# jkk-research/urban_road_filter

Measured on NVIDIA H100. Metric: scans_per_sec, higher is better.
Workload: dtype f32/f64

## Files before the change

### urban_road_filter_b200/csrc/urf_api.cu

```cuda
#include <algorithm>
#include <cmath>
#include <cstdio>
#include <cstdlib>
#include <cstring>
#include <string>
#include <vector>

#include "urf_kernels.cuh"
#include "urf_host.hpp"

using namespace urf;

struct urf_ctx {
  int device = 0;
  int max_points = 0;
  int max_batch = 0;
  size_t P = 0;
  int Tmax = 0;
  cudaStream_t stream = nullptr;
  cudaStream_t s_in = nullptr, s_out = nullptr;
  static constexpr int kGroups = 16;
  cudaStream_t s_grp[kGroups] = {};
  cudaEvent_t ev_fork = nullptr, ev_join[kGroups] = {};
  cudaStream_t s_side[kGroups + 1] = {};
  cudaEvent_t ev_sfork[kGroups + 1] = {}, ev_sjoin[kGroups + 1] = {};
  int sort_ctas = 0;
  int groups = 2;
  bool use_graph = true;
  cudaGraphExec_t gexec = nullptr;
  int g_B = -1, g_S = -1, g_order = -1, g_launches = 0;
  unsigned long long g_version = 0, version = 1;
  std::vector<cudaEvent_t> ev_in, ev_comp;
  cudaEvent_t ev0 = nullptr, ev1 = nullptr;
  DevBuffers buf{};
  float4* own_in = nullptr;
  unsigned char* rawb = nullptr;
  size_t rawb_bytes = 0;
  signed char* label8 = nullptr;
  int* own_label = nullptr;
  float4* pack = nullptr;
  int* packcnt = nullptr;
  int* packtot = nullptr;
  int* h_packtot = nullptr;
  urf_params params{};
  DevParams dp{};
  int* h_n = nullptr;
  static constexpr int kNRing = 8;
  int* h_nring = nullptr;
  cudaEvent_t ev_nring[kNRing] = {};
  int nring_pos = 0;
  ScanOut* h_out = nullptr;
  int last_B = 0, last_S = 0;
  int launches = 0;
  float last_ms = 0.f;
  bool timing_valid = false;
  std::string err;
  std::vector<void*> allocs;
  bool profile = false;
  int kslots = 1, kslot = 0;
  std::vector<cudaEvent_t> kev;
  std::vector<const char*> knames;
  std::vector<int> kcounts;
  int kcount = 0;
};

namespace {

int cuda_rc(urf_ctx* ctx, cudaError_t e, const char* call) {
  if (e == cudaSuccess) return URF_OK;
  ctx->err = std::string(call) + ": " + cudaGetErrorString(e);
  return e == cudaErrorMemoryAllocation ? URF_ERR_NOMEM : URF_ERR_CUDA;
}

#define CK(call)                                                                                   \
  do {                                                                                             \
    const int rc_ = cuda_rc(ctx, (call), #call);                                                   \
    if (rc_ != URF_OK) return rc_;                                                                 \
  } while (0)

template <class T> int dalloc(urf_ctx* ctx, T** p, size_t count) {
  void* q = nullptr;
  CK(cudaMalloc(&q, count * sizeof(T) + 256));
  ctx->allocs.push_back(q);
  CK(cudaMemsetAsync(q, 0, count * sizeof(T) + 256, ctx->stream));
  CK(cudaStreamSynchronize(ctx->stream));
  *p = static_cast<T*>(q);
  return URF_OK;
}

__global__ void k_ring32(DevBuffers buf, int* dst, int S) {
  const int b = blockIdx.y, i = blockIdx.x * blockDim.x + threadIdx.x;
  if (i < buf.n[b]) dst[(size_t)b * S + i] = max((int)buf.ringid[(size_t)b * S + i], -1);
}

DevBuffers offset_view(const DevBuffers& a, int b0, int S, int T, int channels) {
  DevBuffers v = a;
  const size_t o = (size_t)b0 * S;
  v.in += o; v.label += o; v.order += o; v.n += b0; v.out += b0;
  if (v.label8) v.label8 += o;
  v.alpha_v += o; v.mark += o; v.ringid += o; v.sect += o; v.bpt += o;
  v.sr += o; v.sz += o; v.sidx += o; v.ssrz += o; v.ssl += o;
  v.az += o; v.d2 += o; v.baz += o; v.roadlist += o; v.roadcnt += (size_t)b0 * ((S + 31) >> 5); v.sortbuf += 2 * o;
  v.Tf += (size_t)b0 * channels * kTStride; v.Tb += (size_t)b0 * channels * kTStride;
  v.lut += (size_t)b0 * (kElevBins + 1); v.firstidx += (size_t)b0 * (kElevBins + 1);
  v.hist += (size_t)b0 * T * kRingKeys;
  v.cmin += (size_t)b0 * channels * kDegBins; v.cmax += (size_t)b0 * channels * kDegBins;
  v.ne += (size_t)b0 * channels * (kDegBins + 1);
  v.tab += b0;
  return v;
}

constexpr int kMaxKernels = 32;
constexpr int kMarkSingleMax = 300000;
thread_local std::string g_create_err;

int launch_pipeline(urf_ctx* ctx, const DevBuffers& buf, int B, int S, bool want_order, int group, int* launched) {
  DevParams dp = ctx->dp;
  dp.want_order = want_order ? 1 : 0;
  cudaStream_t st = group < urf_ctx::kGroups ? ctx->s_grp[group] : ctx->stream;
  const int T = (S + kChunk - 1) / kChunk;
  if (T > ctx->Tmax) return URF_ERR_CAPACITY;
  int L = 0;
  ctx->kcount = 0;
  const dim3 gpts((S + 255) / 256, B), gchunk((T + kWarpsPerBlock - 1) / kWarpsPerBlock, B);
#define K(name, ...)                                                                         \
  do {                                                                                       \
    if (ctx->profile && ctx->kcount < kMaxKernels) {                                         \
      ctx->knames[ctx->kcount] = name;                                                       \
      CK(cudaEventRecord(ctx->kev[(size_t)ctx->kslot * (kMaxKernels + 1) + ctx->kcount], st)); \
      ctx->kcount++;                                                                         \
    }                                                                                        \
    __VA_ARGS__;                                                                             \
    L++;                                                                                     \
  } while (0)
  K("k_reset", k_reset<<<dim3(8, B), 256, 0, st>>>(buf, dp));
  K("k_points", k_points<<<gpts, 256, 0, st>>>(buf, dp, S));
  K("k_register", k_register<<<B, 256, 0, st>>>(buf, dp, S));
  K("k_assign", k_assign<<<gchunk, kWarpsPerBlock * 32, 0, st>>>(buf, dp, S, T));
  K("k_scan_offsets", k_scan_offsets<<<B, 1024, 0, st>>>(buf, dp, S, T));
  K("k_scatter", k_scatter<<<dim3((T + kScatterWarps - 1) / kScatterWarps, B), kScatterWarps * 32, kScatterSmem, st>>>(buf, dp, S, T));
  const bool fork = dp.star && !ctx->profile;
  cudaStream_t st_ring = fork ? ctx->s_side[group] : st;
  if (fork) {
    CK(cudaEventRecord(ctx->ev_sfork[group], st));
    CK(cudaStreamWaitEvent(st_ring, ctx->ev_sfork[group], 0));
  }
  if (dp.curbPoints == 5)
    K("k_ring_detect4", k_ring_detect4<<<dim3((S + kTile4 - 1) / kTile4, B), 256, 0, st_ring>>>(buf, dp, S));
  else K("k_ring_detect", k_ring_detect<<<gpts, 256, 0, st_ring>>>(buf, dp, S));
  if (fork) CK(cudaEventRecord(ctx->ev_sjoin[group], st_ring));
  if (dp.star) {
    const int gbig = std::max(4, std::min(kSectKeys, 2048 / B));
    const dim3 gscan((kSectKeys + kScanWarps * 32 - 1) / (kScanWarps * 32), B);
    const int gsort = std::min(ctx->sort_ctas, (B * kSectKeys + kSortWarps - 1) / kSortWarps);
    K("k_star_sort", k_star_sort<<<gsort, kSortWarps * 32, kStarSortSmem, st>>>(buf, dp, S, B));
    K("k_star_sort_big", k_star_sort_big<<<dim3(gbig, B), 256, kStarCtaSmem, st>>>(buf, dp, S));
    K("k_star_scan", k_star_scan<<<gscan, kScanWarps * 32, 0, st>>>(buf, dp, S));
    if (dp.star_prefix)
      K("k_star_refine", k_star_refine<<<dim3(std::max(8, std::min(kSectKeys / 8, 8192 / B)), B), 256, kStarCtaSmem, st>>>(buf, dp, S));
  }
  if (fork) CK(cudaStreamWaitEvent(st, ctx->ev_sjoin[group], 0));
  K("k_tab1", k_tab1<<<dim3((dp.channels + 7) / 8, B), 256, 0, st>>>(buf, dp));
  K("k_reach", k_reach<<<dim3((2 * kDegBins + 7) / 8, B), 256, 0, st>>>(buf, dp));
  K("k_tab2", k_tab2<<<dim3((dp.channels + kTab2Rings - 1) / kTab2Rings, B), kTab2Rings * 64, 0, st>>>(buf, dp));
  K("k_label", k_label<<<dim3((S + kLabelThreads * kLabelGroups - 1) / (kLabelThreads * kLabelGroups), B), kLabelThreads, 0, st>>>(buf, dp, S));
  if (S > kMarkSingleMax) {
    const dim3 gm(std::max(1, std::min(64, S / 16384)), B);
    K("k_markers_grid1", k_markers_grid<1><<<gm, kMarkGridThreads, 0, st>>>(buf, S));
    K("k_markers_grid2", k_markers_grid<2><<<gm, kMarkGridThreads, 0, st>>>(buf, S));
    K("k_verts", k_verts<<<B, 384, 0, st>>>(buf, S));
  } else K("k_markers1", k_markers1<<<dim3(1, B), kMark1Threads, 0, st>>>(buf, S));
  if (want_order) K("k_sort_rings", k_sort_rings<<<dim3(dp.channels, B), kSortThreads, kRingSmemKeys * sizeof(unsigned long long), st>>>(buf, S));
#undef K
  if (ctx->profile) {
    CK(cudaEventRecord(ctx->kev[(size_t)ctx->kslot * (kMaxKernels + 1) + kMaxKernels], st));
    ctx->kcounts[ctx->kslot] = ctx->kcount;
    ctx->kslot = (ctx->kslot + 1) % ctx->kslots;
  }
  CK(cudaGetLastError());
  *launched = L;
  return URF_OK;
}

int update_graph(urf_ctx* ctx, int B, int S, bool want_order) {
  if (ctx->gexec && ctx->g_B == B && ctx->g_S == S && ctx->g_order == (int)want_order && ctx->g_version == ctx->version) return URF_OK;
  if (ctx->gexec) { cudaGraphExecDestroy(ctx->gexec); ctx->gexec = nullptr; }
  cudaGraph_t graph = nullptr;
  CK(cudaStreamBeginCapture(ctx->stream, cudaStreamCaptureModeThreadLocal));
  int L = 0;
  const int rc = launch_pipeline(ctx, ctx->buf, B, S, want_order, urf_ctx::kGroups, &L);
  const cudaError_t e = cudaStreamEndCapture(ctx->stream, &graph);
  if (rc != URF_OK || e != cudaSuccess || !graph) { if (graph) cudaGraphDestroy(graph); ctx->err = "graph capture failed"; return rc != URF_OK ? rc : URF_ERR_CUDA; }
  const cudaError_t ei = cudaGraphInstantiate(&ctx->gexec, graph, 0);
  cudaGraphDestroy(graph);
  if (ei != cudaSuccess) { ctx->gexec = nullptr; ctx->err = cudaGetErrorString(ei); return URF_ERR_CUDA; }
  ctx->g_B = B; ctx->g_S = S; ctx->g_order = (int)want_order; ctx->g_version = ctx->version; ctx->g_launches = L;
  return URF_OK;
}

void fill_result(const ScanOut& o, urf_result* r, bool with_ring_start) {
  r->n_in = o.n_in; r->n_roi = o.n_roi;
  r->flags = o.flags & F_PUBLIC_MASK; r->reserved = 0;
  if (o.n_roi < 30) {
    r->status = URF_TOO_FEW_POINTS;
    r->n_rings = 0; r->n_order = 0; r->n_road = 0; r->n_curb = 0; r->n_vert = 0;
    if (with_ring_start && r->ring_start) for (int k = 0; k <= URF_MAX_CHANNELS; k++) r->ring_start[k] = 0;
    return;
  }
  r->status = URF_OK;
  r->n_rings = o.n_rings; r->n_order = o.n_order; r->n_road = o.n_road; r->n_curb = o.n_curb; r->n_vert = o.n_vert;
  std::memcpy(r->vert, o.vert, sizeof(float) * 4 * (size_t)o.n_vert);
  if (with_ring_start && r->ring_start) std::memcpy(r->ring_start, o.ring_start, sizeof(int) * (URF_MAX_CHANNELS + 1));
}

}

extern "C" {

int urf_version(void) { return URF_VERSION; }

const char* urf_strerror(int code) {
  switch (code) {
    case URF_OK: return "ok";
    case URF_TOO_FEW_POINTS: return "fewer than 30 points in the ROI: nothing published";
    case URF_ERR_INVALID: return "invalid argument";
    case URF_ERR_NO_DEVICE: return "no CUDA device (this library has no CPU fallback)";
    case URF_ERR_CUDA: return "CUDA error";
    case URF_ERR_NOMEM: return "out of device or pinned memory";
    case URF_ERR_CAPACITY: return "scan or batch larger than the context was created for";
    case URF_ERR_TIMEOUT: return "timed out";
    case URF_ERR_CLOSED: return "queue closed";
    default: return "unknown error";
  }
}

const char* urf_last_cuda_error(const urf_ctx* ctx) {
  if (ctx) return ctx->err.c_str();
  return g_create_err.empty() ? "null context" : g_create_err.c_str();
}

void urf_default_params(urf_params* p) {
  if (!p) return;
  std::memset(p, 0, sizeof(*p));
  std::snprintf(p->fixed_frame, sizeof(p->fixed_frame), "left_os1/os1_lidar");
  std::snprintf(p->topic_name, sizeof(p->topic_name), "/left_os1/os1_cloud_node/points");
  p->x_zero_method = 1; p->z_zero_method = 1; p->star_shaped_method = 1; p->blind_spots = 1; p->xDirection = 0;
  p->interval = 0.18; p->curb_height = 0.05; p->curb_points = 5; p->beamZone = 30;
  p->min_x = 0; p->max_x = 30; p->min_y = -10; p->max_y = 10; p->min_z = -3; p->max_z = -1;
  p->cylinder_deg_x = 150; p->cylinder_deg_z = 140; p->curb_slope_deg = 50;
  p->kdev_param = 1.225; p->kdist_param = 2; p->starbeam_filter = 0; p->dmin_param = 10;
  p->simple_poly_allow = 1; p->poly_s_param = 0.7; p->poly_z_manual = -1.5; p->poly_z_avg_allow = 1;
  p->channels = 64;
}

int urf_create(urf_ctx** out, int device, int max_points, int max_batch) {
  if (!out || max_points < 1 || max_batch < 1 || max_points > (1 << 24)) return URF_ERR_INVALID;
  if ((long long)(max_points + kChunk) * max_batch >= (1ll << 31)) return URF_ERR_CAPACITY;
  *out = nullptr;
  int ndev = 0;
  if (cudaGetDeviceCount(&ndev) != cudaSuccess || ndev <= 0 || device < 0 || device >= ndev) return URF_ERR_NO_DEVICE;
  urf_ctx* ctx = new urf_ctx();
  auto fail = [&](int rc) { g_create_err = ctx->err.empty() ? std::string(urf_strerror(rc)) : ctx->err; urf_destroy(ctx); return rc; };
  ctx->device = device;
  if (cudaSetDevice(device) != cudaSuccess) return fail(URF_ERR_NO_DEVICE);
  ctx->max_points = ((max_points + kChunk - 1) / kChunk) * kChunk;
  ctx->max_batch = max_batch;
  ctx->P = (size_t)ctx->max_points * max_batch;
  ctx->Tmax = ctx->max_points / kChunk;
  int rc;
#define TRY(x) do { rc = (x); if (rc != URF_OK) return fail(rc); } while (0)
#define CKF(call) do { cudaError_t e_ = (call); if (e_ != cudaSuccess) { ctx->err = cudaGetErrorString(e_); return fail(URF_ERR_CUDA); } } while (0)
  CKF(cudaStreamCreateWithFlags(&ctx->stream, cudaStreamNonBlocking));
  CKF(cudaStreamCreateWithFlags(&ctx->s_in, cudaStreamNonBlocking));
  CKF(cudaStreamCreateWithFlags(&ctx->s_out, cudaStreamNonBlocking));
  for (int g = 0; g < urf_ctx::kGroups; g++) {
    CKF(cudaStreamCreateWithFlags(&ctx->s_grp[g], cudaStreamNonBlocking));
    CKF(cudaEventCreateWithFlags(&ctx->ev_join[g], cudaEventDisableTiming));
  }
  CKF(cudaEventCreateWithFlags(&ctx->ev_fork, cudaEventDisableTiming));
  for (int g = 0; g <= urf_ctx::kGroups; g++) {
    CKF(cudaStreamCreateWithFlags(&ctx->s_side[g], cudaStreamNonBlocking));
    CKF(cudaEventCreateWithFlags(&ctx->ev_sfork[g], cudaEventDisableTiming));
    CKF(cudaEventCreateWithFlags(&ctx->ev_sjoin[g], cudaEventDisableTiming));
  }
  CKF(cudaEventCreate(&ctx->ev0));
  CKF(cudaEventCreate(&ctx->ev1));
  const size_t P = ctx->P;
  DevBuffers& b = ctx->buf;
  TRY(dalloc(ctx, &ctx->own_in, P));
  ctx->rawb_bytes = (size_t)ctx->max_points * URF_MAX_POINT_STEP;
  TRY(dalloc(ctx, &ctx->rawb, ctx->rawb_bytes));
  TRY(dalloc(ctx, &b.alpha_v, P));
  TRY(dalloc(ctx, &b.mark, P));
  TRY(dalloc(ctx, &b.ringid, P));
  TRY(dalloc(ctx, &b.sect, P));
  TRY(dalloc(ctx, &ctx->own_label, P));
  TRY(dalloc(ctx, &b.bpt, P));
  TRY(dalloc(ctx, &b.sr, P));
  TRY(dalloc(ctx, &b.sz, P));
  TRY(dalloc(ctx, &b.sidx, P));
  TRY(dalloc(ctx, &b.ssrz, P));
  TRY(dalloc(ctx, &b.ssl, P));
  TRY(dalloc(ctx, &b.az, P));
  TRY(dalloc(ctx, &b.d2, P));
  TRY(dalloc(ctx, &b.baz, P));
  TRY(dalloc(ctx, &b.roadlist, P));
  TRY(dalloc(ctx, &b.roadcnt, P / 32 + (size_t)max_batch + 1));
  TRY(dalloc(ctx, &b.Tf, (size_t)max_batch * kTStride * URF_MAX_CHANNELS));
  TRY(dalloc(ctx, &b.Tb, (size_t)max_batch * kTStride * URF_MAX_CHANNELS));
  TRY(dalloc(ctx, &b.lut, (size_t)max_batch * (kElevBins + 1)));
  TRY(dalloc(ctx, &b.order, P));
  TRY(dalloc(ctx, &b.sortbuf, 2 * P));
  TRY(dalloc(ctx, &b.hist, (size_t)max_batch * ctx->Tmax * kRingKeys));
  TRY(dalloc(ctx, &b.firstidx, (size_t)max_batch * (kElevBins + 1)));
  TRY(dalloc(ctx, &b.cmin, (size_t)max_batch * URF_MAX_CHANNELS * kDegBins));
  TRY(dalloc(ctx, &b.cmax, (size_t)max_batch * URF_MAX_CHANNELS * kDegBins));
  TRY(dalloc(ctx, &b.ne, (size_t)max_batch * URF_MAX_CHANNELS * (kDegBins + 1)));
  TRY(dalloc(ctx, &b.newY, (size_t)ctx->max_points));
  TRY(dalloc(ctx, &b.n, (size_t)max_batch));
  TRY(dalloc(ctx, &b.out, (size_t)max_batch));
  TRY(dalloc(ctx, &b.tab, (size_t)max_batch));
  b.in = ctx->own_in;
  b.label = ctx->own_label;
  CKF(cudaMallocHost((void**)&ctx->h_n, sizeof(int) * max_batch));
  CKF(cudaMallocHost((void**)&ctx->h_nring, sizeof(int) * max_batch * urf_ctx::kNRing));
  for (int r = 0; r < urf_ctx::kNRing; r++) CKF(cudaEventCreateWithFlags(&ctx->ev_nring[r], cudaEventDisableTiming));
  CKF(cudaMallocHost((void**)&ctx->h_out, sizeof(ScanOut) * max_batch));
  {
    std::vector<float> ny;
    host_newY(ny, ctx->max_points);
    CKF(cudaMemcpy(b.newY, ny.data(), sizeof(float) * ny.size(), cudaMemcpyHostToDevice));
    float bd[kSectKeys], bo[kSectKeys], Kfi;
    unsigned char byx[kSectKeys];
    host_beam_init(bd, bo, byx, &Kfi);
    CKF(cudaMemcpyToSymbol(c_beam_d, bd, sizeof(bd)));
    CKF(cudaMemcpyToSymbol(c_beam_o, bo, sizeof(bo)));
    CKF(cudaMemcpyToSymbol(c_beam_yx, byx, sizeof(byx)));
    ctx->dp.Kfi = Kfi;
  }
  CKF(cudaFuncSetAttribute(k_star_sort, cudaFuncAttributeMaxDynamicSharedMemorySize, (int)kStarSortSmem));
  {
    int sms = 0, per_sm = 0;
    CKF(cudaDeviceGetAttribute(&sms, cudaDevAttrMultiProcessorCount, ctx->device));
    CKF(cudaOccupancyMaxActiveBlocksPerMultiprocessor(&per_sm, k_star_sort, kSortWarps * 32, kStarSortSmem));
    ctx->sort_ctas = std::max(1, sms * per_sm);
  }
  CKF(cudaFuncSetAttribute(k_star_sort_big, cudaFuncAttributeMaxDynamicSharedMemorySize, (int)kStarCtaSmem));
  CKF(cudaFuncSetAttribute(k_star_refine, cudaFuncAttributeMaxDynamicSharedMemorySize, (int)kStarCtaSmem));
  CKF(cudaFuncSetAttribute(k_scatter, cudaFuncAttributeMaxDynamicSharedMemorySize, (int)kScatterSmem));
  CKF(cudaFuncSetAttribute(k_scatter, cudaFuncAttributePreferredSharedMemoryCarveout, (int)cudaSharedmemCarveoutMaxShared));
  CKF(cudaFuncSetAttribute(k_sort_rings, cudaFuncAttributeMaxDynamicSharedMemorySize, (int)(kRingSmemKeys * sizeof(unsigned long long))));
  urf_default_params(&ctx->params);
  const char* fe = std::getenv("URF_FORCE_EXACT_REGISTRATION");
  narrow_params(&ctx->params, &ctx->dp, ctx->dp.Kfi, fe && fe[0] == '1', 0);
  const char* sp = std::getenv("URF_STAR_PREFIX");
  ctx->dp.star_prefix = !(sp && sp[0] == '0');
  ctx->dp.star_pivot = 17;
#undef TRY
#undef CKF
  *out = ctx;
  return URF_OK;
}

void urf_destroy(urf_ctx* ctx) {
  if (!ctx) return;
  cudaSetDevice(ctx->device);
  if (ctx->stream) cudaStreamSynchronize(ctx->stream);
  for (void* p : ctx->allocs) cudaFree(p);
  if (ctx->h_n) cudaFreeHost(ctx->h_n);
  if (ctx->h_nring) cudaFreeHost(ctx->h_nring);
  for (cudaEvent_t e : ctx->ev_nring) if (e) cudaEventDestroy(e);
  if (ctx->h_out) cudaFreeHost(ctx->h_out);
  if (ctx->h_packtot) cudaFreeHost(ctx->h_packtot);
  if (ctx->gexec) cudaGraphExecDestroy(ctx->gexec);
  for (cudaEvent_t e : ctx->kev) cudaEventDestroy(e);
  for (cudaEvent_t e : ctx->ev_in) cudaEventDestroy(e);
  for (cudaEvent_t e : ctx->ev_comp) cudaEventDestroy(e);
  for (int g = 0; g < urf_ctx::kGroups; g++) { if (ctx->s_grp[g]) cudaStreamDestroy(ctx->s_grp[g]); if (ctx->ev_join[g]) cudaEventDestroy(ctx->ev_join[g]); }
  if (ctx->ev_fork) cudaEventDestroy(ctx->ev_fork);
  for (int g = 0; g <= urf_ctx::kGroups; g++) {
    if (ctx->s_side[g]) cudaStreamDestroy(ctx->s_side[g]);
    if (ctx->ev_sfork[g]) cudaEventDestroy(ctx->ev_sfork[g]);
    if (ctx->ev_sjoin[g]) cudaEventDestroy(ctx->ev_sjoin[g]);
  }
  if (ctx->s_in) cudaStreamDestroy(ctx->s_in);
  if (ctx->s_out) cudaStreamDestroy(ctx->s_out);
  if (ctx->ev0) cudaEventDestroy(ctx->ev0);
  if (ctx->ev1) cudaEventDestroy(ctx->ev1);
  if (ctx->stream) cudaStreamDestroy(ctx->stream);
  delete ctx;
}

void* urf_pinned_alloc(size_t bytes) {
  void* p = nullptr;
  if (cudaHostAlloc(&p, bytes ? bytes : 1, cudaHostAllocPortable) != cudaSuccess) { cudaGetLastError(); return nullptr; }
  return p;
}
void urf_pinned_free(void* p) { if (p) cudaFreeHost(p); }

int urf_set_params(urf_ctx* ctx, const urf_params* p) {
  if (!ctx || !p) return URF_ERR_INVALID;
  int rc = validate_params(p);
  if (rc != URF_OK) return rc;
  ctx->params = *p;
  narrow_params(p, &ctx->dp, ctx->dp.Kfi, ctx->dp.force_exact, 0);
  ctx->version++;
  return URF_OK;
}

int urf_get_params(const urf_ctx* ctx, urf_params* p) {
  if (!ctx || !p) return URF_ERR_INVALID;
  *p = ctx->params;
  return URF_OK;
}

int urf_set_option(urf_ctx* ctx, int option, int value) {
  if (!ctx) return URF_ERR_INVALID;
  CK(cudaSetDevice(ctx->device));
  ctx->version++;
  if (option == 0) { ctx->dp.force_exact = value != 0; ctx->version++; return URF_OK; }
  if (option == 4) { ctx->dp.star_prefix = value != 0; ctx->version++; return URF_OK; }
  if (option == 3) { ctx->use_graph = value != 0; return URF_OK; }
  if (option == 2) { ctx->groups = value < 1 ? 1 : (value > urf_ctx::kGroups ? urf_ctx::kGroups : value); return URF_OK; }
  if ((option >= 5 && option <= 9) || option == 11 || option == 12) return URF_OK;
  if (option == 10) { ctx->dp.star_pivot = value < 3 ? 3 : (value > 28 ? 28 : value); return URF_OK; }
  if (option == 1) {
    CK(cudaStreamSynchronize(ctx->stream));
    if (ctx->gexec) { cudaGraphExecDestroy(ctx->gexec); ctx->gexec = nullptr; ctx->g_B = -1; }
    for (cudaEvent_t e : ctx->kev) cudaEventDestroy(e);
    ctx->kev.clear();
    ctx->profile = value > 0;
    ctx->kslots = value > 0 ? value : 1;
    ctx->kslot = 0;
    if (ctx->profile) {
      ctx->kev.assign((size_t)ctx->kslots * (kMaxKernels + 1), nullptr);
      for (cudaEvent_t& e : ctx->kev) {
        const cudaError_t ce = cudaEventCreate(&e);
        if (ce != cudaSuccess) {
          for (cudaEvent_t f : ctx->kev) if (f) cudaEventDestroy(f);
          ctx->kev.clear(); ctx->profile = false; ctx->kslots = 1;
          ctx->err = std::string("cudaEventCreate: ") + cudaGetErrorString(ce);
          return URF_ERR_CUDA;
// ... 311 lines not shown
```

### urban_road_filter_b200/csrc/urf_kernels.cuh

```cuda
#pragma once
#include <type_traits>

#include "urf_device.cuh"
#include "urf_logic.cuh"
#include "urf_stdsort.cuh"

namespace urf {

__constant__ float c_beam_d[kSectKeys];
__constant__ float c_beam_o[kSectKeys];
__constant__ unsigned char c_beam_yx[kSectKeys];

__device__ __forceinline__ int lane_id() { return threadIdx.x & 31; }
__device__ __forceinline__ unsigned scan_base(int b, int S) { return (unsigned)b * (unsigned)S; }

template <class T>
__device__ void cta_bitonic(T* a, int npad) {
  for (int k = 2; k <= npad; k <<= 1) {
    for (int j = k >> 1; j > 0; j >>= 1) {
      for (int t = threadIdx.x; t < (npad >> 1); t += blockDim.x) {
        int i = 2 * t - (t & (j - 1));
        int l = i + j;
        bool up = (i & k) == 0;
        T x = a[i], y = a[l];
        if ((x > y) == up) { a[i] = y; a[l] = x; }
      }
      __syncthreads();
    }
  }
}

__device__ __forceinline__ int next_pow2(int n) { int p = 1; while (p < n) p <<= 1; return p; }

__device__ __forceinline__ void curb_hit(const DevBuffers& buf, const DevParams& prm, int b, unsigned gb, int idx, int k) {
  buf.mark[gb + (unsigned)idx] = 2;
  if (k < 0) k = buf.ringid[gb + (unsigned)idx];
  if (k < 0) return;
  const float a = buf.az[gb + (unsigned)idx];
  if (a >= 0.0f) {
    const unsigned o = ((unsigned)b * (unsigned)prm.channels + (unsigned)k) * kDegBins + (unsigned)deg_bin(a);
    atomicMin(&buf.cmin[o], fbits(a));
    atomicMax(&buf.cmax[o], fbits(a));
  }
}
__device__ __forceinline__ int ring_of_position(const int* __restrict__ ring_start, int p) {
  int lo = 0, hi = kRingKeys;
  while (lo < hi) { const int mid = (lo + hi) >> 1; if (ring_start[mid] <= p) lo = mid + 1; else hi = mid; }
  return lo - 1;
}

__global__ void k_reset(DevBuffers buf, DevParams prm) {
  const int b = blockIdx.y;
  const int tid = blockIdx.x * blockDim.x + threadIdx.x;
  const int nth = gridDim.x * blockDim.x;
  ScanOut& o = buf.out[b];
  ScanTab& t = buf.tab[b];
  if (tid == 0) {
    o.n_in = buf.n[b]; o.n_roi = 0; o.n_rings = 0; o.n_order = 0; o.n_road = 0; o.n_curb = 0; o.n_vert = 0; o.flags = 0;
  }
  for (int i = tid; i <= kRingKeys; i += nth) o.ring_start[i] = 0;
  for (int i = tid; i < kRingKeys; i += nth) { t.maxs[i] = 0ull; t.maxdist[i] = 0u; t.angle[i] = 0.f; t.regidx[i] = 0x7fffffff; t.regorder[i] = 0x7fffffff; }
  for (int i = tid; i < kDegBins; i += nth) { t.cutbest[i] = ~0ull; t.dmax[i] = 0u; t.best[i] = ~0ull; }
  for (int i = tid; i < kSectKeys; i += nth) t.sect_cnt[i] = 0;
  if (tid == 0) { t.nbig = 0; t.nslow = 0; t.nrefine = 0; }
  unsigned* fi = buf.firstidx + (size_t)b * (kElevBins + 1);
  for (int i = tid; i <= kElevBins; i += nth) fi[i] = 0xffffffffu;
  const size_t nb = (size_t)prm.channels * kDegBins;
  unsigned* cmin = buf.cmin + (size_t)b * nb;
  unsigned* cmax = buf.cmax + (size_t)b * nb;
  for (size_t i = tid; i < nb; i += nth) { cmin[i] = 0x7f800000u; cmax[i] = 0u; }
}

__global__ void __launch_bounds__(256) k_points(DevBuffers buf, DevParams prm, int S) {
  const int b = blockIdx.y;
  const int n = buf.n[b];
  const int i = blockIdx.x * blockDim.x + threadIdx.x;
  int keep = 0, sec = -1;
  if (i < n) {
    const unsigned g = scan_base(b, S) + (unsigned)i;
    const float4 p = __ldg(&buf.in[g]);
    keep = roi_keep(prm, p.x, p.y, p.z);
    float a = -1.0f;
    if (keep) {
      float d, az;
      point_angles(p.x, p.y, p.z, &a, &d, &az);
      unsigned* fi = buf.firstidx + (size_t)b * (kElevBins + 1) + elev_bin(a);
      if (*fi > (unsigned)i) atomicMin(fi, (unsigned)i);
      if (a == 0.0f) atomicOr(&buf.out[b].flags, F_ZERO_ALPHA);
      if (az != az) atomicOr(&buf.out[b].flags, F_NAN_AZIMUTH);
      if (prm.star) sec = star_sector(prm, p.x, p.y, c_beam_d, c_beam_o, c_beam_yx);
      buf.az[g] = az;
      buf.d2[g] = d;
    }
    buf.alpha_v[g] = a;
    buf.mark[g] = 0;
    buf.sect[g] = (short)sec;
  }
  const unsigned bal = __ballot_sync(0xffffffffu, keep);
  if (lane_id() == 0 && bal) atomicAdd(&buf.out[b].n_roi, __popc(bal));
  const unsigned peers = __match_any_sync(0xffffffffu, sec);
  if (sec >= 0 && lane_id() == __ffs(peers) - 1) atomicAdd(&buf.tab[b].sect_cnt[sec], __popc(peers));
}

__device__ void register_exact_cta(const float* __restrict__ alpha, int n, float interval, int channels, float* s_vis,
                                   float* s_reg, int* s_idx, int* s_red, int* out_m) {
  __shared__ int s_min;
  int m = 0, vis = 0, i_last = -1;
  bool frozen = false;
  while (m < channels) {
    int local = 0x7fffffff;
    for (int i = i_last + 1 + threadIdx.x; i < n; i += blockDim.x) {
      const float a = alpha[i];
      if (a < 0.0f) continue;
      bool cov = false;
      for (int t = 0; t < vis; t++) {
        if (fabsf(__fsub_rn(s_vis[t], a)) <= interval) { cov = true; break; }
      }
      if (!cov) { local = i; break; }
    }
    for (int o = 16; o > 0; o >>= 1) local = min(local, __shfl_xor_sync(0xffffffffu, local, o));
    if (lane_id() == 0) s_red[threadIdx.x >> 5] = local;
    __syncthreads();
    if (threadIdx.x == 0) {
      int v = 0x7fffffff;
      for (int w = 0; w < (int)(blockDim.x >> 5); w++) v = min(v, s_red[w]);
      s_min = v;
    }
    __syncthreads();
    const int istar = s_min;
    __syncthreads();
    if (istar == 0x7fffffff) break;
    const float a = alpha[istar];
    if (threadIdx.x == 0) { s_reg[m] = a; s_idx[m] = istar; if (!frozen && a != 0.0f) s_vis[vis] = a; }
    if (!frozen) { if (a == 0.0f) frozen = true; else vis++; }
    m++;
    i_last = istar;
    __syncthreads();
  }
  *out_m = m;
}

__device__ void publish_rings_cta(ScanTab& tab, ScanOut& out, unsigned short* lut, float interval, const float* s_reg,
                                  const int* s_idx, int m, unsigned long long* s_keys, float* s_sorted) {
  for (int t = threadIdx.x; t < kRingKeys; t += blockDim.x)
    s_keys[t] = t < m ? (((unsigned long long)fbits(s_reg[t]) << 32) | (unsigned)s_idx[t]) : ~0ull;
  __syncthreads();
  cta_bitonic(s_keys, kRingKeys);
  for (int t = threadIdx.x; t < kRingKeys; t += blockDim.x) {
    if (t < m) {
      const float a = bitsf((unsigned)(s_keys[t] >> 32));
      s_sorted[t] = a;
      tab.angle[t] = a;
      tab.regidx[t] = (int)(unsigned)s_keys[t];
      tab.regorder[t] = s_idx[t];
    } else { s_sorted[t] = 0.f; tab.angle[t] = 0.f; tab.regidx[t] = 0x7fffffff; tab.regorder[t] = 0x7fffffff; }
  }
  if (threadIdx.x == 0) out.n_rings = m;
  __syncthreads();
  for (int e = threadIdx.x; e <= kElevBins; e += blockDim.x) lut[e] = (unsigned short)ring_lut_entry(s_sorted, m, interval, e);
}

__global__ void __launch_bounds__(256) k_register(DevBuffers buf, DevParams prm, int S) {
  const int b = blockIdx.x;
  const int n = buf.n[b];
  ScanOut& out = buf.out[b];
  ScanTab& tab = buf.tab[b];
  const float* alpha = buf.alpha_v + (size_t)b * S;
  __shared__ unsigned s_cand[kMaxCand];
  __shared__ float s_calpha[kMaxCand];
  __shared__ float s_vis[kRingKeys];
  __shared__ float s_reg[kRingKeys];
  __shared__ float s_sorted[kRingKeys];
  __shared__ int s_idx[kRingKeys];
  __shared__ unsigned long long s_keys[kRingKeys];
  __shared__ int s_red[8];
  __shared__ int s_cnt, s_m;
  if (out.n_roi < 30) {
    if (threadIdx.x == 0) out.n_rings = 0;
    return;
  }
  bool exact = prm.force_exact || (out.flags & F_ZERO_ALPHA);
  if (!exact) {
    if (threadIdx.x == 0) s_cnt = 0;
    __syncthreads();
    const unsigned* fi = buf.firstidx + (size_t)b * (kElevBins + 1);
    for (int t = threadIdx.x; t <= kElevBins; t += blockDim.x) {
      const unsigned v = fi[t];
      if (v != 0xffffffffu) { int s = atomicAdd(&s_cnt, 1); if (s < kMaxCand) s_cand[s] = v; }
    }
    __syncthreads();
    const int cnt = s_cnt;
    if (cnt > kMaxCand) exact = true;
    else {
      const int npad = next_pow2(cnt < 2 ? 2 : cnt);
      for (int t = cnt + threadIdx.x; t < npad; t += blockDim.x) s_cand[t] = 0xffffffffu;
      __syncthreads();
      cta_bitonic(s_cand, npad);
      for (int t = threadIdx.x; t < cnt; t += blockDim.x) s_calpha[t] = alpha[s_cand[t]];
      __syncthreads();
      if (threadIdx.x < 32) {
        int m = 0;
        for (int c = 0; c < cnt && m < prm.channels; c++) {
          const float a = s_calpha[c];
          bool cov = false;
          for (int t = lane_id(); t < m; t += 32)
            if (fabsf(__fsub_rn(s_reg[t], a)) <= prm.interval) cov = true;
          cov = __any_sync(0xffffffffu, cov);
          if (!cov) {
            if (lane_id() == 0) { s_reg[m] = a; s_idx[m] = (int)s_cand[c]; }
            m++;
            __syncwarp();
          }
        }
        if (lane_id() == 0) s_m = m;
      }
      __syncthreads();
    }
  }
  if (exact) {
    int m;
    register_exact_cta(alpha, n, prm.interval, prm.channels, s_vis, s_reg, s_idx, s_red, &m);
    if (threadIdx.x == 0) { s_m = m; atomicOr(&out.flags, F_EXACT_REG); }
    __syncthreads();
  }
  publish_rings_cta(tab, out, buf.lut + (size_t)b * (kElevBins + 1), prm.interval, s_reg, s_idx, s_m, s_keys, s_sorted);
}

__device__ __forceinline__ bool assign_chunk(const DevBuffers& buf, const DevParams& prm, int b, int S, int T, int chunk, int n, bool live,
                                             bool verify, const float* s_angle, const int* s_regidx, const int* regorder, int R,
                                             const unsigned short* __restrict__ lut, unsigned* cnt, int lane) {
  bool violation = false;
  constexpr int H = 8;
  static_assert((kChunk / 32) % H == 0, "chunk iterations come in groups of H");
#pragma unroll 1
  for (int h0 = 0; h0 < kChunk / 32; h0 += H) {
    float av[H];
    unsigned short start[H];
#pragma unroll
    for (int u = 0; u < H; u++) {
      const int i = chunk * kChunk + (h0 + u) * 32 + lane;
      av[u] = i < n ? buf.alpha_v[scan_base(b, S) + (unsigned)i] : -1.0f;
    }
#pragma unroll
    for (int u = 0; u < H; u++) start[u] = (live && av[u] >= 0.0f) ? lut[elev_bin(av[u])] : (unsigned short)0;
#pragma unroll
    for (int u = 0; u < H; u++) {
      const int i = chunk * kChunk + (h0 + u) * 32 + lane;
      int ring = -1;
      if (i < n) {
        const float a = av[u];
        const bool kept = live && a >= 0.0f;
        if (kept) {
          int lo;
          ring = assign_ring_from(s_angle, R, a, prm.interval, start[u], &lo);
          if (verify && registration_violation(s_angle, s_regidx, regorder, R, prm.channels, prm.interval, a, i, lo)) violation = true;
        }
        buf.ringid[scan_base(b, S) + (unsigned)i] = kept ? (short)ring : (short)-2;
      }
      const int ring0 = __shfl_sync(0xffffffffu, ring, 0);
      if (__all_sync(0xffffffffu, ring == ring0)) { if (lane == 0 && ring0 >= 0) atomicAdd(&cnt[ring0], 32u); }
      else if (ring >= 0) atomicAdd(&cnt[ring], 1u);
    }
  }
  __syncwarp();
  unsigned* row = buf.hist + ((size_t)b * T + chunk) * kRingKeys;
  for (int t = lane; t < kRingKeys; t += 32) row[t] = cnt[t];
  return violation;
}

__global__ void __launch_bounds__(kWarpsPerBlock * 32) k_assign(DevBuffers buf, DevParams prm, int S, int T) {
  const int b = blockIdx.y;
  ScanOut& out = buf.out[b];
  const int flags = out.flags;
  const int n = buf.n[b];
  const int warp = threadIdx.x >> 5, lane = lane_id();
  const int chunk = blockIdx.x * kWarpsPerBlock + warp;
  __shared__ float s_angle[kRingKeys];
  __shared__ int s_regidx[kRingKeys];
  __shared__ unsigned s_cnt[kWarpsPerBlock][kRingKeys];
  ScanTab& tab = buf.tab[b];
  const int R = out.n_rings;
  for (int t = threadIdx.x; t < kRingKeys; t += blockDim.x) { s_angle[t] = tab.angle[t]; s_regidx[t] = tab.regidx[t]; }
  for (int t = lane; t < kRingKeys; t += 32) s_cnt[warp][t] = 0;
  __syncthreads();
  if (chunk * kChunk >= n) return;
  const bool violation = assign_chunk(buf, prm, b, S, T, chunk, n, out.n_roi >= 30, !(flags & F_EXACT_REG), s_angle, s_regidx, tab.regorder, R,
                                      buf.lut + (size_t)b * (kElevBins + 1), s_cnt[warp], lane);
  if (__any_sync(0xffffffffu, violation) && lane == 0) atomicOr(&out.flags, F_SPEC_VIOLATION);
}

__global__ void __launch_bounds__(1024) k_scan_offsets(DevBuffers buf, DevParams prm, int S, int T) {
  __shared__ unsigned s_part[32][kRingKeys];
  __shared__ unsigned s_base[kRingKeys];
  const int b = blockIdx.x;
  const int n = buf.n[b];
  const int rows = (n + kChunk - 1) / kChunk;
  const int warp = threadIdx.x >> 5, lane = lane_id();
  {
    ScanOut& out = buf.out[b];
    const int flags = out.flags;
    if ((flags & F_SPEC_VIOLATION) && !(flags & F_EXACT_REG)) {
      __shared__ float s_vis[kRingKeys], s_reg[kRingKeys], s_sorted[kRingKeys];
      __shared__ int s_idx[kRingKeys];
      __shared__ unsigned long long s_keys[kRingKeys];
      __shared__ int s_red[32];
      __shared__ int s_m;
      int m;
      register_exact_cta(buf.alpha_v + (size_t)b * S, n, prm.interval, prm.channels, s_vis, s_reg, s_idx, s_red, &m);
      if (threadIdx.x == 0) s_m = m;
      __syncthreads();
      const unsigned short* lut = buf.lut + (size_t)b * (kElevBins + 1);
      publish_rings_cta(buf.tab[b], out, buf.lut + (size_t)b * (kElevBins + 1), prm.interval, s_reg, s_idx, s_m, s_keys, s_sorted);
      __syncthreads();
      const int R = s_m;
      for (int c0 = 0; c0 < rows; c0 += 32) {
        for (int t = lane; t < kRingKeys; t += 32) s_part[warp][t] = 0;
        __syncwarp();
        if (c0 + warp < rows) assign_chunk(buf, prm, b, S, T, c0 + warp, n, true, false, s_sorted, nullptr, nullptr, R, lut, s_part[warp], lane);
        __syncwarp();
      }
      if (threadIdx.x == 0) out.flags = flags | F_EXACT_REG;
      __syncthreads();
    }
  }
  const int rpw = (rows + 31) / 32;
  const int r0 = min(rows, warp * rpw), r1 = min(rows, (warp + 1) * rpw);
  unsigned* hist = buf.hist + (size_t)b * T * kRingKeys;
  for (int key = lane; key < kRingKeys; key += 32) {
    unsigned s = 0;
    for (int r = r0; r < r1; r++) s += hist[(size_t)r * kRingKeys + key];
    s_part[warp][key] = s;
  }
  __syncthreads();
  if (threadIdx.x < kRingKeys) {
    unsigned run = 0;
    for (int w = 0; w < 32; w++) { unsigned v = s_part[w][threadIdx.x]; s_part[w][threadIdx.x] = run; run += v; }
    s_base[threadIdx.x] = run;
  }
  __syncthreads();
  if (threadIdx.x == 0) {
    unsigned run = 0;
    ScanOut& o = buf.out[b];
    for (int k = 0; k < kRingKeys; k++) { unsigned v = s_base[k]; s_base[k] = run; o.ring_start[k] = (int)run; run += v; }
    o.ring_start[kRingKeys] = (int)run;
    o.n_order = (int)run;
  } else if (threadIdx.x == 32) {
    ScanTab& t = buf.tab[b];
    int run = 0;
    for (int k = 0; k < kSectKeys; k++) { const int v = t.sect_cnt[k]; t.sect_start[k] = run; t.sect_cur[k] = run; run += v; }
    t.sect_start[kSectKeys] = run;
  }
  __syncthreads();
  for (int key = lane; key < kRingKeys; key += 32) {
    unsigned run = s_base[key] + s_part[warp][key];
    for (int r = r0; r < r1; r++) {
      unsigned* p = &hist[(size_t)r * kRingKeys + key];
      unsigned v = *p; *p = run; run += v;
    }
  }
}

__device__ __forceinline__ void mbar_init(unsigned long long* bar, unsigned count) {
  asm volatile("mbarrier.init.shared::cta.b64 [%0], %1;\n" ::"r"((unsigned)__cvta_generic_to_shared(bar)), "r"(count) : "memory");
  asm volatile("fence.proxy.async.shared::cta;\n" ::: "memory");
}
__device__ __forceinline__ void bulk_copy_g2s(void* dst, const void* src, unsigned bytes, unsigned long long* bar) {
  const unsigned d = (unsigned)__cvta_generic_to_shared(dst), m = (unsigned)__cvta_generic_to_shared(bar);
  asm volatile("mbarrier.arrive.expect_tx.shared::cta.b64 _, [%0], %1;\n" ::"r"(m), "r"(bytes) : "memory");
  asm volatile("cp.async.bulk.shared::cluster.global.mbarrier::complete_tx::bytes [%0], [%1], %2, [%3];\n"
               ::"r"(d), "l"(src), "r"(bytes), "r"(m) : "memory");
}
__device__ __forceinline__ void mbar_wait(unsigned long long* bar, unsigned phase) {
  const unsigned m = (unsigned)__cvta_generic_to_shared(bar);
  unsigned done;
  do {
    asm volatile("{\n .reg .pred p;\n mbarrier.try_wait.parity.shared::cta.b64 p, [%1], %2;\n selp.u32 %0, 1, 0, p;\n}\n"
                 : "=r"(done) : "r"(m), "r"(phase) : "memory");
  } while (!done);
}
constexpr int kScatterWarps = 4;
constexpr size_t kScatterSmem = (size_t)kScatterWarps * kChunk * sizeof(float4);
__global__ void __launch_bounds__(kScatterWarps * 32, 4) k_scatter(DevBuffers buf, DevParams prm, int S, int T) {
  const int b = blockIdx.y;
  const int n = buf.n[b];
  const int warp = threadIdx.x >> 5, lane = lane_id();
  const int chunk = blockIdx.x * kScatterWarps + warp;
  extern __shared__ float4 s_tiles[];
  __shared__ unsigned long long s_bar[kScatterWarps];
  __shared__ unsigned s_delta[kScatterWarps][kChunk];
  __shared__ unsigned s_lcnt[kScatterWarps][kRingKeys];
  __shared__ unsigned short s_perm[kScatterWarps][kChunk];
  __shared__ int s_scnt[kSectKeys], s_sbase[kSectKeys];
  const float4* tile = s_tiles + warp * kChunk;
  unsigned* delta = s_delta[warp];
  unsigned* lcnt = s_lcnt[warp];
  unsigned short* perm = s_perm[warp];
  ScanTab& tab = buf.tab[b];
  const bool live = chunk * kChunk < n;
  const unsigned* row = buf.hist + ((size_t)b * T + chunk) * kRingKeys;
  const unsigned gb = scan_base(b, S), g0 = gb + (unsigned)chunk * kChunk;
  if (live && lane == 0) {
    mbar_init(&s_bar[warp], 1);
    bulk_copy_g2s(s_tiles + warp * kChunk, buf.in + g0, (unsigned)min(kChunk, n - chunk * kChunk) * sizeof(float4), &s_bar[warp]);
  }
  for (int t = threadIdx.x; t < kSectKeys; t += blockDim.x) s_scnt[t] = 0;
  for (int t = lane; t < kRingKeys; t += 32) lcnt[t] = 0;
  __syncthreads();
  const unsigned lt = (1u << lane) - 1u;
  unsigned packed[kChunk / 32];
  unsigned spack[kChunk / 32];
  if (live) {
    constexpr int GRP = kChunk / 32;
#pragma unroll
    for (int h = 0; h < kChunk / 32 / GRP; h++) {
      short rr[GRP], ss[GRP];
#pragma unroll
      for (int u = 0; u < GRP; u++) {
        const int li = (h * GRP + u) * 32 + lane;
        const bool in = chunk * kChunk + li < n;
        rr[u] = in ? buf.ringid[g0 + li] : (short)-1;
        ss[u] = in ? buf.sect[g0 + li] : (short)-1;
      }
#pragma unroll
      for (int u = 0; u < GRP; u++) {
        const int it = h * GRP + u;
        const int sec = ss[u];
        const int sec0 = __shfl_sync(0xffffffffu, sec, 0);
        int srank = 0;
        if (__all_sync(0xffffffffu, sec == sec0)) {
          int sb = 0;
          if (lane == 0 && sec0 >= 0) sb = atomicAdd(&s_scnt[sec0], 32);
          srank = __shfl_sync(0xffffffffu, sb, 0) + lane;
        } else if (sec >= 0) srank = atomicAdd(&s_scnt[sec], 1);
        spack[it] = sec >= 0 ? (((unsigned)(sec + 1) << 16) | (unsigned)srank) : 0u;
        const int ring = rr[u];
        const int rprev = __shfl_up_sync(0xffffffffu, ring, 1), ring0 = __shfl_sync(0xffffffffu, ring, 0);
        unsigned peers;
        if (__all_sync(0xffffffffu, ring == ring0)) peers = 0xffffffffu;
        else if (__all_sync(0xffffffffu, lane == 0 || ring > rprev) || __all_sync(0xffffffffu, lane == 0 || ring < rprev)) peers = 1u << lane;
        else peers = __match_any_sync(0xffffffffu, ring);
        const int leader = __ffs(peers) - 1;
        unsigned rb = 0;
        if (ring >= 0 && lane == leader) rb = atomicAdd(&lcnt[ring], (unsigned)__popc(peers));
        rb = __shfl_sync(0xffffffffu, rb, leader);
        packed[it] = ring >= 0 ? (((unsigned)(ring + 1) << 16) | (rb + __popc(peers & lt))) : 0u;
      }
    }
  }
  __syncthreads();
  for (int t = threadIdx.x; t < kSectKeys; t += blockDim.x) {
    const int c = s_scnt[t];
    s_sbase[t] = c > 0 ? atomicAdd(&tab.sect_cur[t], c) : 0;
  }
  int total = 0;
  if (live) {
    {
      unsigned v[kRingKeys / 32], sum = 0;
#pragma unroll
      for (int j = 0; j < kRingKeys / 32; j++) { v[j] = lcnt[lane * (kRingKeys / 32) + j]; sum += v[j]; }
      unsigned inc = sum;
      for (int o = 1; o < 32; o <<= 1) { unsigned t = __shfl_up_sync(0xffffffffu, inc, o); if (lane >= o) inc += t; }
      unsigned run = inc - sum;
      __syncwarp();
#pragma unroll
      for (int j = 0; j < kRingKeys / 32; j++) { lcnt[lane * (kRingKeys / 32) + j] = run; run += v[j]; }
    }
    __syncwarp();
#pragma unroll
    for (int it = 0; it < kChunk / 32; it++) {
      const unsigned pk = packed[it];
      if (pk) {
        const int ring = (int)(pk >> 16) - 1;
        const unsigned lstart = lcnt[ring];
        const int slot = lstart + (pk & 0xffffu);
        perm[slot] = (unsigned short)(it * 32 + lane);
        delta[slot] = __ldg(&row[ring]) - lstart;
      }
      total += __popc(__ballot_sync(0xffffffffu, pk != 0));
    }
    __syncwarp();
    mbar_wait(&s_bar[warp], 0);
    for (int t = lane; t < total; t += 32) {
      const int li = perm[t];
      const float4 p = tile[li];
      const unsigned dst = gb + delta[t] + (unsigned)t;
      buf.bpt[dst] = make_float4(p.x, p.y, p.z, __int_as_float(chunk * kChunk + li));
      if (prm.want_order) buf.baz[dst] = make_uint2(fbits(buf.az[g0 + li]), (unsigned)(chunk * kChunk + li));
    }
  }
  __syncthreads();
  if (live) {
#pragma unroll
    for (int it = 0; it < kChunk / 32; it++) {
      const unsigned sp = spack[it];
      if (sp) {
        const int sec = (int)(sp >> 16) - 1;
        const int li = it * 32 + lane;
        const float4 p = tile[li];
        const unsigned dst = gb + (unsigned)(s_sbase[sec] + (int)(sp & 0xffffu));
        buf.sr[dst] = star_radius(p.x, p.y);
        buf.sz[dst] = p.z;
        buf.sidx[dst] = (unsigned)(chunk * kChunk + li);
      }
    }
  }
}

constexpr int kWarpCap = 1024, kCtaCap = 8192;
constexpr int kNetCap = 512;
constexpr unsigned kSslIndex = 0x80000000u;

struct SectorRecs {
  const DevBuffers& buf;
  unsigned o;
  unsigned at;
  __device__ __forceinline__ const float* r() const { return buf.sr + o; }
  __device__ __forceinline__ unsigned key(int e) const { return fbits(buf.sr[o + (unsigned)e]); }
  __device__ __forceinline__ void put(int e, unsigned k, unsigned slot) const {
    buf.ssrz[at + (unsigned)e] = make_float2(bitsf(k), buf.sz[o + slot]);
    buf.ssl[at + (unsigned)e] = slot;
  }
};
__device__ __forceinline__ SectorRecs sector_recs(const DevBuffers& buf, int b, int S, int base, int at = 0) {
  const unsigned o = scan_base(b, S) + (unsigned)base;
  return SectorRecs{buf, o, o + (unsigned)at};
}
__device__ __forceinline__ int star_input_index(const DevBuffers& buf, unsigned o, int e) {
  const unsigned l = buf.ssl[o + (unsigned)e];
  return (l & kSslIndex) ? (int)(l & ~kSslIndex) : (int)buf.sidx[o + l];
}

template <int EPL, int WARPS, bool LIST = false, bool STAGED = false>
__device__ __forceinline__ bool bitonic_sector(const SectorRecs& d, int n, int tid, unsigned* s_xk, unsigned* s_xe) {
  constexpr int THREADS = WARPS * 32;
  const int lane = tid & 31;
  unsigned key[EPL], el[EPL];
#pragma unroll
  for (int r = 0; r < EPL; r++) {
    const int e = tid * EPL + r;
    key[r] = 0xffffffffu; el[r] = 0u;
    if (e < n) {
      if (LIST) { key[r] = s_xk[e]; el[r] = (STAGED && s_xe == nullptr) ? (unsigned)e : s_xe[e]; }
      else { key[r] = d.key(e); el[r] = (unsigned)e; }
    }
  }
  auto intra = [&](int k_over_epl, auto kc) {
    constexpr int K = decltype(kc)::value;
#pragma unroll
    for (int j = (K > 0 ? K : EPL) >> 1; j > 0; j >>= 1) {
#pragma unroll
      for (int r = 0; r < EPL; r++) {
        if ((r & j) == 0) {
          const bool asc = K > 0 ? ((r & K) == 0) : ((tid & k_over_epl) == 0);
          const bool sw = (key[r] > key[r | j]) == asc;
          const unsigned ka = sw ? key[r | j] : key[r], kb = sw ? key[r] : key[r | j];
          const unsigned ea = sw ? el[r | j] : el[r], eb = sw ? el[r] : el[r | j];
          key[r] = ka; key[r | j] = kb; el[r] = ea; el[r | j] = eb;
        }
      }
    }
  };
  if (EPL > 2) intra(0, std::integral_constant<int, 2>());
  if (EPL > 4) intra(0, std::integral_constant<int, 4>());
  if (EPL > 8) intra(0, std::integral_constant<int, 8>());
  if (EPL > 16) intra(0, std::integral_constant<int, 16>());
  for (int ke = 1; ke <= THREADS; ke <<= 1) {
    for (int tj = ke >> 1; tj > 0; tj >>= 1) {
      const bool keep_min = ((tid & tj) == 0) == ((tid & ke) == 0);
      if (tj < 32) {
#pragma unroll
        for (int r = 0; r < EPL; r++) {
          const unsigned o = __shfl_xor_sync(0xffffffffu, key[r], tj);
          const unsigned oe = __shfl_xor_sync(0xffffffffu, el[r], tj);
          const bool take = (o < key[r]) == keep_min;
          key[r] = take ? o : key[r];
          el[r] = take ? oe : el[r];
        }
      } else {
        __syncthreads();
#pragma unroll
        for (int r = 0; r < EPL; r++) { s_xk[r * THREADS + tid] = key[r]; s_xe[r * THREADS + tid] = el[r]; }
        __syncthreads();
#pragma unroll
        for (int r = 0; r < EPL; r++) {
          const unsigned o = s_xk[r * THREADS + (tid ^ tj)], oe = s_xe[r * THREADS + (tid ^ tj)];
          const bool take = (o < key[r]) == keep_min;
          key[r] = take ? o : key[r];
          el[r] = take ? oe : el[r];
        }
      }
    }
    intra(ke, std::integral_constant<int, 0>());
  }
  unsigned prev0 = __shfl_up_sync(0xffffffffu, key[EPL - 1], 1);
  if (WARPS > 1) {
    __syncthreads();
    if (lane == 31) s_xk[tid >> 5] = key[EPL - 1];
    __syncthreads();
    if (lane == 0 && tid > 0) prev0 = s_xk[(tid >> 5) - 1];
  }
  bool tie = false;
  if constexpr (STAGED) {
    static_assert(!STAGED || (WARPS == 1 && LIST && EPL <= 16), "STAGED: single-warp list sorts of up to 16 elements per lane");
#pragma unroll
    for (int r = 0; r < EPL; r++) {
      const int e = tid * EPL + r;
      const unsigned prev = r > 0 ? key[r - 1] : prev0;
      if (e < n && e > 0 && prev == key[r]) tie = true;
    }
    static_assert(!STAGED || 32 * EPL <= kNetCap, "STAGED: the keys go kNetCap words above the slots");
    constexpr int TPW = 32 / EPL;
    __syncwarp();
#pragma unroll
    for (int r = 0; r < EPL; r++) {
      const int w = tid * EPL + (r ^ ((tid / TPW) & (EPL - 1)));
      s_xk[w] = el[r];
      s_xk[kNetCap + w] = key[r];
    }
    __syncwarp();
#pragma unroll
    for (int r = 0; r < EPL; r++) {
      const int e = r * 32 + tid, t = e / EPL;
      const int w = t * EPL + ((e & (EPL - 1)) ^ ((t / TPW) & (EPL - 1)));
      if (e < n) d.put(e, s_xk[kNetCap + w], s_xk[w]);
    }
    __syncwarp();
  } else {
#pragma unroll
    for (int r = 0; r < EPL; r++) {
      const int e = tid * EPL + r;
      const unsigned prev = r > 0 ? key[r - 1] : prev0;
      if (e < n) {
        d.put(e, key[r], el[r]);
        if (e > 0 && prev == key[r]) tie = true;
      }
    }
  }
  return tie;
}

__device__ __forceinline__ bool near_prefix(int m, int n) { return m >= 32 && 4 * m <= 3 * n; }

template <int EPL>
__device__ __forceinline__ int select_near(unsigned* kb, int n, int lane, int pivot_rank) {
  const unsigned mine = kb[(int)(((unsigned)lane * (unsigned)n) >> 5)];
  unsigned key[EPL];
#pragma unroll
  for (int r = 0; r < EPL; r++) {
    const int e = r * 32 + lane;
    key[r] = e < n ? kb[e] : 0xffffffffu;
  }
  int rank = 0;
#pragma unroll
  for (int j = 0; j < 32; j++) { const unsigned o = __shfl_sync(0xffffffffu, mine, j); rank += (o < mine) || (o == mine && j < lane); }
  const unsigned pivot = __shfl_sync(0xffffffffu, mine, __ffs(__ballot_sync(0xffffffffu, rank == pivot_rank)) - 1);
  int m = 0;
#pragma unroll
  for (int r = 0; r < EPL; r++) m += __popc(__ballot_sync(0xffffffffu, key[r] < pivot));
  if (!near_prefix(m, n) || m > kNetCap) return m;
  __syncwarp();
  const unsigned lt = (1u << lane) - 1u;
  int pos0 = 0;
#pragma unroll
  for (int r = 0; r < EPL; r++) {
    const bool sel = key[r] < pivot;
    const unsigned bs = __ballot_sync(0xffffffffu, sel);
    const int pos = pos0 + __popc(bs & lt);
    if (sel) { kb[pos] = key[r]; kb[kNetCap + pos] = (unsigned)(r * 32 + lane); }
    pos0 += __popc(bs);
  }
  __syncwarp();
  return m;
}

template <int EPL>
__device__ __forceinline__ int select_far(const float* __restrict__ sr, int n, int lane, unsigned* s_pk, unsigned* s_pe, unsigned kmax) {
  unsigned key[EPL];
#pragma unroll
  for (int r = 0; r < EPL; r++) {
    const int e = r * 32 + lane;
    key[r] = e < n ? fbits(sr[e]) : 0u;
  }
  const unsigned lt = (1u << lane) - 1u;
  int m = 0;
#pragma unroll
  for (int r = 0; r < EPL; r++) {
    const bool sel = key[r] > kmax;
    const unsigned bs = __ballot_sync(0xffffffffu, sel);
    if (sel) { const int pos = m + __popc(bs & lt); s_pk[pos] = key[r]; s_pe[pos] = (unsigned)(r * 32 + lane); }
    m += __popc(bs);
  }
  __syncwarp();
  return m;
}

constexpr int kPrefixMin = 128;

__device__ __forceinline__ void cp_async4(unsigned* s, const float* g) {
  asm volatile("cp.async.ca.shared.global [%0], [%1], 4;\n" ::"r"((unsigned)__cvta_generic_to_shared(s)), "l"(g) : "memory");
}
__device__ __forceinline__ void cp_async16(unsigned* s, const float* g) {
  asm volatile("cp.async.cg.shared.global [%0], [%1], 16;\n" ::"r"((unsigned)__cvta_generic_to_shared(s)), "l"(g) : "memory");
// ... 1197 lines not shown
```

Baseline: 78430.

## Compact ring histogram to channel stride and parallelize offset scan

Shrinks the per-chunk ring histogram stride from kRingKeys to the actual channel count, cutting memory traffic in assign, scan_offsets and scatter. Rewrites k_scan_offsets to use 512 threads with batched loads that expose memory-level parallelism. It also replaces the serial single-thread prefix sums over ring and sector keys with warp-shuffle block scans. This relies on channels being at most kRingKeys and consistently used as the stride across all kernels.

```diff
diff --git a/urban_road_filter_b200/csrc/urf_api.cu b/urban_road_filter_b200/csrc/urf_api.cu
--- a/urban_road_filter_b200/csrc/urf_api.cu
+++ b/urban_road_filter_b200/csrc/urf_api.cu
@@ -103,7 +103,7 @@
   v.az += o; v.d2 += o; v.baz += o; v.roadlist += o; v.roadcnt += (size_t)b0 * ((S + 31) >> 5); v.sortbuf += 2 * o;
   v.Tf += (size_t)b0 * channels * kTStride; v.Tb += (size_t)b0 * channels * kTStride;
   v.lut += (size_t)b0 * (kElevBins + 1); v.firstidx += (size_t)b0 * (kElevBins + 1);
-  v.hist += (size_t)b0 * T * kRingKeys;
+  v.hist += (size_t)b0 * T * channels;
   v.cmin += (size_t)b0 * channels * kDegBins; v.cmax += (size_t)b0 * channels * kDegBins;
   v.ne += (size_t)b0 * channels * (kDegBins + 1);
   v.tab += b0;
@@ -137,7 +137,7 @@
   K("k_points", k_points<<<gpts, 256, 0, st>>>(buf, dp, S));
   K("k_register", k_register<<<B, 256, 0, st>>>(buf, dp, S));
   K("k_assign", k_assign<<<gchunk, kWarpsPerBlock * 32, 0, st>>>(buf, dp, S, T));
-  K("k_scan_offsets", k_scan_offsets<<<B, 1024, 0, st>>>(buf, dp, S, T));
+  K("k_scan_offsets", k_scan_offsets<<<B, kScanOffThreads, 0, st>>>(buf, dp, S, T));
   K("k_scatter", k_scatter<<<dim3((T + kScatterWarps - 1) / kScatterWarps, B), kScatterWarps * 32, kScatterSmem, st>>>(buf, dp, S, T));
   const bool fork = dp.star && !ctx->profile;
   cudaStream_t st_ring = fork ? ctx->s_side[group] : st;
diff --git a/urban_road_filter_b200/csrc/urf_kernels.cuh b/urban_road_filter_b200/csrc/urf_kernels.cuh
--- a/urban_road_filter_b200/csrc/urf_kernels.cuh
+++ b/urban_road_filter_b200/csrc/urf_kernels.cuh
@@ -263,8 +263,9 @@
     }
   }
   __syncwarp();
-  unsigned* row = buf.hist + ((size_t)b * T + chunk) * kRingKeys;
-  for (int t = lane; t < kRingKeys; t += 32) row[t] = cnt[t];
+  const int C = prm.channels;
+  unsigned* row = buf.hist + ((size_t)b * T + chunk) * C;
+  for (int t = lane; t < C; t += 32) row[t] = cnt[t];
   return violation;
 }
 
@@ -289,11 +290,16 @@
   if (__any_sync(0xffffffffu, violation) && lane == 0) atomicOr(&out.flags, F_SPEC_VIOLATION);
 }
 
-__global__ void __launch_bounds__(1024) k_scan_offsets(DevBuffers buf, DevParams prm, int S, int T) {
-  __shared__ unsigned s_part[32][kRingKeys];
+constexpr int kScanOffThreads = 512, kScanOffWarps = kScanOffThreads / 32;
+constexpr int kScanOffBatch = 16;
+static_assert(kRingKeys < kScanOffThreads && kSectKeys <= kScanOffThreads, "one ring_start entry and one sector per thread");
+__global__ void __launch_bounds__(kScanOffThreads, 2) k_scan_offsets(DevBuffers buf, DevParams prm, int S, int T) {
+  __shared__ unsigned s_part[kScanOffWarps][kRingKeys];
   __shared__ unsigned s_base[kRingKeys];
+  __shared__ unsigned s_wsum[2][kScanOffWarps];
   const int b = blockIdx.x;
   const int n = buf.n[b];
+  const int C = prm.channels;
   const int rows = (n + kChunk - 1) / kChunk;
   const int warp = threadIdx.x >> 5, lane = lane_id();
   {
@@ -313,7 +319,7 @@
       publish_rings_cta(buf.tab[b], out, buf.lut + (size_t)b * (kElevBins + 1), prm.interval, s_reg, s_idx, s_m, s_keys, s_sorted);
       __syncthreads();
       const int R = s_m;
-      for (int c0 = 0; c0 < rows; c0 += 32) {
+      for (int c0 = 0; c0 < rows; c0 += kScanOffWarps) {
         for (int t = lane; t < kRingKeys; t += 32) s_part[warp][t] = 0;
         __syncwarp();
         if (c0 + warp < rows) assign_chunk(buf, prm, b, S, T, c0 + warp, n, true, false, s_sorted, nullptr, nullptr, R, lut, s_part[warp], lane);
@@ -323,39 +329,57 @@
       __syncthreads();
     }
   }
-  const int rpw = (rows + 31) / 32;
+  ScanTab& tab = buf.tab[b];
+  const unsigned scnt = threadIdx.x < kSectKeys ? (unsigned)tab.sect_cnt[threadIdx.x] : 0u;
+  const int rpw = (rows + kScanOffWarps - 1) / kScanOffWarps;
   const int r0 = min(rows, warp * rpw), r1 = min(rows, (warp + 1) * rpw);
-  unsigned* hist = buf.hist + (size_t)b * T * kRingKeys;
-  for (int key = lane; key < kRingKeys; key += 32) {
+  unsigned* hist = buf.hist + (size_t)b * T * C;
+  for (int key = lane; key < C; key += 32) {
     unsigned s = 0;
-    for (int r = r0; r < r1; r++) s += hist[(size_t)r * kRingKeys + key];
+    for (int r = r0; r < r1; r += kScanOffBatch) {
+      unsigned v[kScanOffBatch];
+#pragma unroll
+      for (int u = 0; u < kScanOffBatch; u++) v[u] = r + u < r1 ? hist[(size_t)(r + u) * C + key] : 0u;
+#pragma unroll
+      for (int u = 0; u < kScanOffBatch; u++) s += v[u];
+    }
     s_part[warp][key] = s;
   }
   __syncthreads();
-  if (threadIdx.x < kRingKeys) {
-    unsigned run = 0;
-    for (int w = 0; w < 32; w++) { unsigned v = s_part[w][threadIdx.x]; s_part[w][threadIdx.x] = run; run += v; }
-    s_base[threadIdx.x] = run;
-  }
-  __syncthreads();
-  if (threadIdx.x == 0) {
-    unsigned run = 0;
-    ScanOut& o = buf.out[b];
-    for (int k = 0; k < kRingKeys; k++) { unsigned v = s_base[k]; s_base[k] = run; o.ring_start[k] = (int)run; run += v; }
-    o.ring_start[kRingKeys] = (int)run;
-    o.n_order = (int)run;
-  } else if (threadIdx.x == 32) {
-    ScanTab& t = buf.tab[b];
-    int run = 0;
-    for (int k = 0; k < kSectKeys; k++) { const int v = t.sect_cnt[k]; t.sect_start[k] = run; t.sect_cur[k] = run; run += v; }
-    t.sect_start[kSectKeys] = run;
-  }
-  __syncthreads();
-  for (int key = lane; key < kRingKeys; key += 32) {
+  unsigned rtot = 0;
+  if (threadIdx.x < C)
+    for (int w = 0; w < kScanOffWarps; w++) { const unsigned v = s_part[w][threadIdx.x]; s_part[w][threadIdx.x] = rtot; rtot += v; }
+  unsigned xr = rtot, xs = scnt;
+#pragma unroll
+  for (int d = 1; d < 32; d <<= 1) {
+    const unsigned ur = __shfl_up_sync(0xffffffffu, xr, d), us = __shfl_up_sync(0xffffffffu, xs, d);
+    if (lane >= d) { xr += ur; xs += us; }
+  }
+  if (lane == 31) { s_wsum[0][warp] = xr; s_wsum[1][warp] = xs; }
+  __syncthreads();
+  unsigned all_r = 0, all_s = 0;
+#pragma unroll
+  for (int w = 0; w < kScanOffWarps; w++) {
+    const unsigned ur = s_wsum[0][w], us = s_wsum[1][w];
+    if (w < warp) { xr += ur; xs += us; }
+    all_r += ur; all_s += us;
+  }
+  xr -= rtot; xs -= scnt;
+  ScanOut& o = buf.out[b];
+  if (threadIdx.x < C) s_base[threadIdx.x] = xr;
+  if (threadIdx.x <= kRingKeys) o.ring_start[threadIdx.x] = (int)(threadIdx.x < C ? xr : all_r);
+  if (threadIdx.x < kSectKeys) { tab.sect_start[threadIdx.x] = (int)xs; tab.sect_cur[threadIdx.x] = (int)xs; }
+  if (threadIdx.x == 0) { o.n_order = (int)all_r; tab.sect_start[kSectKeys] = (int)all_s; }
+  __syncthreads();
+  for (int key = lane; key < C; key += 32) {
     unsigned run = s_base[key] + s_part[warp][key];
-    for (int r = r0; r < r1; r++) {
-      unsigned* p = &hist[(size_t)r * kRingKeys + key];
-      unsigned v = *p; *p = run; run += v;
+    for (int r = r0; r < r1; r += kScanOffBatch) {
+      unsigned v[kScanOffBatch];
+#pragma unroll
+      for (int u = 0; u < kScanOffBatch; u++) v[u] = r + u < r1 ? hist[(size_t)(r + u) * C + key] : 0u;
+#pragma unroll
+      for (int u = 0; u < kScanOffBatch; u++)
+        if (r + u < r1) { hist[(size_t)(r + u) * C + key] = run; run += v[u]; }
     }
   }
 }
@@ -397,7 +421,7 @@
   unsigned short* perm = s_perm[warp];
   ScanTab& tab = buf.tab[b];
   const bool live = chunk * kChunk < n;
-  const unsigned* row = buf.hist + ((size_t)b * T + chunk) * kRingKeys;
+  const unsigned* row = buf.hist + ((size_t)b * T + chunk) * prm.channels;
   const unsigned gb = scan_base(b, S), g0 = gb + (unsigned)chunk * kChunk;
   if (live && lane == 0) {
     mbar_init(&s_bar[warp], 1);
```

Result: faster. 82180, median of 6 (+4.8%).
